# evfro/polara

Hardware: AMD Instinct MI355X
Metric: users scored/sec + SVD build time, ML-20M rank-50 PureSVD (higher is better)
Workload: dtype bf16x3; 1 GPU; ML-20M-shaped synthetic 138493 x 26744, ~2e7 nnz, 10 levels (BASELINE.json metric / configs[2]), PureSVD rank=50, top-10, all users scored; n_items=26744, nnz=19975287, rank=50, topk=10, prune=True, launch=python, passes on 2 streams

## Files before the change

include/polara_hip.h:

```cpp
#ifndef POLARA_HIP_H
#define POLARA_HIP_H

#include <stdint.h>

#ifdef __cplusplus
extern "C" {
#endif

#define PK_OK 0
#define PK_E_INVALID (-1)
#define PK_E_LAUNCH (-2)
#define PK_E_UNSUPPORTED (-3)
#define PK_E_NOCONV (-4)

#define PK_VAL_F32 0
#define PK_VAL_F64 1

const char *pk_last_error(void);
int pk_version(void);
int pk_set_option(const char *name, int32_t value, int32_t unset);
int pk_copy_to_host_async(void *stream, void *dst_host, const void *src_dev, int64_t bytes);
int pk_device_info(int device, char *name, int name_len, int *cu_count, int64_t *hbm_bytes);
int pk_warm_up(void);

// ... 171 lines not shown
                            const int64_t *task_end_dev, const int32_t *task_slot_dev, int64_t n_long,
                            const int32_t *long_row_dev, const int32_t *long_slot_begin_dev,
                            const int32_t *long_slot_end_dev, const int32_t *indices_dev, const void *vals_dev,
                            int val_kind, const double *X_dev, int64_t ldx, int32_t nc, double *out_dev, int64_t ldo,
                            double *partial_dev, int64_t x_rows, const int32_t *row_flags_dev, int32_t flag_mask);

int pk_spmm_csr_rows_list_f64(void *stream, int64_t cap, const int32_t *list_dev, const int32_t *count_dev, int64_t row_offset,
                              const int64_t *row_first_task_dev, const int32_t *task_row_dev, const int64_t *task_begin_dev,
                              const int64_t *task_end_dev, const int32_t *task_slot_dev, int64_t n_long,
                              const int32_t *long_row_dev, const int32_t *long_slot_begin_dev, const int32_t *long_slot_end_dev,
                              const int32_t *indices_dev, const void *vals_dev, int val_kind, const double *X_dev, int64_t ldx,
                              int32_t nc, double *out_dev, int64_t ldo, double *partial_dev, int64_t x_rows,
                              const int32_t *row_flags_dev, int32_t flag_mask);

int32_t pk_q20_lanes(int32_t K);
double pk_q20_kappa(int32_t K);
int64_t pk_q20_image_bytes(int64_t n, int32_t K);
int pk_q20_encode_f64(void *stream, int64_t n, int32_t K, const double *V_dev, int64_t ldv, void *img_dev,
                      double *tab_dev, void *work_dev, int32_t *info_dev);
int pk_q20_decode_f64(void *stream, int64_t n, int32_t K, const void *img_dev, const double *tab_dev, double *out_dev,
                      int64_t ldo);
int pk_fold_q20(void *stream, int64_t n_tasks, const int32_t *task_row_dev, const int64_t *task_begin_dev,
                const int64_t *task_end_dev, const int32_t *task_slot_dev, int64_t n_long,
                const int32_t *long_row_dev, const int32_t *long_slot_begin_dev, const int32_t *long_slot_end_dev,
                const int32_t *indices_dev, const void *vals_dev, int val_kind, const void *img_dev,
                const double *tab_dev, int64_t n_items, int32_t K, int32_t Kx, double *out_dev, int64_t ldo,
                double *partial_dev);
int pk_fold_q20_zero(void *stream, int64_t n_tasks, const int32_t *task_row_dev, const int64_t *task_begin_dev,
                     const int64_t *task_end_dev, const int32_t *task_slot_dev, int64_t n_long,
                     const int32_t *long_row_dev, const int32_t *long_slot_begin_dev, const int32_t *long_slot_end_dev,
                     const int32_t *indices_dev, const void *vals_dev, int val_kind, const void *img_dev,
                     const double *tab_dev, int64_t n_items, int32_t K, int32_t Kx, double *out_dev, int64_t ldo,
                     double *partial_dev, int32_t *zero_dev, int32_t zero_n);
int pk_scatter_rows_i64(void *stream, int64_t n_rows, int32_t width, const int64_t *src_dev, const int64_t *perm_dev,
                        int64_t *dst);
int pk_map_ids_i64(void *stream, int64_t n, const int64_t *src_dev, const int64_t *table_dev, int64_t n_table, int64_t *dst);
int64_t pk_exact_work_bytes(int32_t n_rows, int64_t n_items);
int pk_score_exact_rows_f64(void *stream, int32_t n_rows, const int32_t *rows_dev, int64_t n_items,
                            int32_t K, const double *V_dev, int64_t ldv, const double *E_dev, int64_t lde,
                            const int64_t *seen_ptr_dev, const int32_t *seen_idx_dev, int32_t topk,
                            int64_t *out_idx_dev, double *out_score_dev, void *work_dev);
int pk_exact_work_init(void *stream, void *work_dev, int32_t n_rows, int64_t n_items);
int pk_score_exact_list_f64(void *stream, int32_t n_wg, const int32_t *list_dev, const int32_t *count_dev, int64_t n_items,
                            int32_t K, const double *V_dev, int64_t ldv, const double *E_dev, int64_t lde,
                            const int64_t *seen_ptr_dev, const int32_t *seen_idx_dev, int32_t topk, int64_t *out_idx_dev,
                            double *out_score_dev, void *work_dev, const int64_t *out_perm_dev);
int pk_eval_ranks(void *stream, int64_t n_holdout, const int64_t *recs_dev, int32_t topk,
                  const int64_t *hold_row_dev, const int64_t *hold_item_dev, int32_t *rank_out_dev);
int32_t pk_eval_cols(void);
int pk_eval_user_metrics(void *stream, int64_t n_users, int32_t topk, const int64_t *recs_dev, int64_t ld,
                         const int64_t *hold_ptr_dev, const int64_t *hold_item_dev, const double *hold_rel_dev,
                         const unsigned char *hold_pos_dev, double not_rated_penalty, double switch_positive,
                         int32_t alternative, double *out_dev);
int64_t pk_eval_reduce_work_bytes(int64_t n_users);
int pk_eval_reduce(void *stream, int64_t n_users, const double *table_dev, double *sums_dev, void *work_dev);
int pk_unique_count_i64(void *stream, int64_t n, const int64_t *ids_dev, int64_t n_bins, int32_t *flags_dev,
                        int64_t *count_dev);
int pk_dense_scores_f64(void *stream, int32_t n_rows, int64_t n_items, int32_t K, const double *V_dev,
                        int64_t ldv, const double *E_dev, int64_t lde, double *out_dev, int64_t ldo);
int pk_topk_rows_f64(void *stream, int64_t n_rows, int64_t n_cols, const double *scores_dev, int64_t ld, int32_t topk,
                     int64_t *out_idx_dev);

int32_t pk_i2i_max_topk(void);
int32_t pk_i2i_window(void);
int32_t pk_i2i_build_window(void);
int64_t pk_i2i_ld(int64_t n_items);
// ... 302 lines not shown
```

polara_amd/_lib.py:

```python
import ctypes as C
import os

_HERE = os.path.dirname(os.path.abspath(__file__))
LIB_PATH = os.environ.get('POLARA_HIP_LIB') or os.path.join(_HERE, 'libpolarahip.so')

PK_VAL_F32, PK_VAL_F64 = 0, 1
PK_KNN_SCALE, PK_KNN_COSINE, PK_KNN_TANIMOTO = 0, 1, 2
PK_PMF_MAX_BLOCKS = 4096
PK_WARP_MAX_SAMPLED = 64
PK_SPLIT_ASCENDING, PK_SPLIT_RANDOM_LO, PK_SPLIT_NO_ORDER, PK_SPLIT_POS_ASCENDING = 1, 2, 4, 8

_vp, _i32, _i64, _f64 = C.c_void_p, C.c_int32, C.c_int64, C.c_double


class PkSweepSettle(C.Structure):
    _fields_ = [('topk', _i32), ('vmax', _f64), ('item_norm', _vp), ('out_idx', _vp), ('out_perm', _vp), ('flags', _vp),
                ('open_list', _vp), ('open_count', _vp)]


PROTOTYPES = {
    'pk_last_error': (C.c_char_p, []),
    'pk_version': (C.c_int, []),
    'pk_warm_up': (C.c_int, []),
    'pk_device_info': (C.c_int, [C.c_int, C.c_char_p, C.c_int, C.POINTER(C.c_int), C.POINTER(_i64)]),
# ... 43 lines not shown
    'pk_pack_frag_f32': (C.c_int, [_vp, _i64, _i32, _vp, _i64, _vp]),
    'pk_candidate_capacity': (_i32, [_i32]),
    'pk_score_state_bytes': (_i64, [_i64, _i32]),
    'pk_score_splits': (_i32, [_i64, _i32]),
    'pk_seen_tiles_build': (C.c_int, [_vp, _i64, _vp, _vp, _i32, _i64, _vp, _vp]),
    'pk_seen_tiles_max_unsorted_row': (_i32, []),
    'pk_score_candidates_f32': (C.c_int, [_vp, _i64, _i64, _i32, _vp, _vp, _vp, _vp, _i64, _vp, _i64, _f64, _vp, _vp, _vp, _vp,
                                          _i32, _i32, _vp, _vp, _vp, _i32, _vp, _vp, _vp, _i32, C.POINTER(PkSweepSettle)]),
    'pk_sweep_settles': (C.c_int, [_i32]),
    'pk_score_two_phase_plan': (C.c_int, [_i64, _i64, _i32, _vp, _vp]),
    'pk_score_two_phase_f32': (C.c_int, [_vp, _i64, _i64, _i32, _vp, _vp, _vp, _vp, _i64, _vp, _i64, _f64, _vp, _vp, _vp, _vp,
                                         _i32, _i32, _i32, _vp, _vp, _vp, _vp, _vp, _i32, _vp, _vp, _vp, _i32]),
    'pk_seen_dense_bytes': (_i64, [_i64, _i32]),
    'pk_seen_dense_build': (C.c_int, [_vp, _i64, _vp, _vp, _vp, _i32, _vp, _vp]),
    'pk_score_chunk_launches': (_i32, [_i64, _i32, _i32, _i32, _i32]),
    'pk_pack_frag_bound_f32': (C.c_int, [_vp, _i64, _i32, _vp, _i64, _vp, _vp, _vp, _i64, _f64]),
    'pk_row_norm_bound_f32': (C.c_int, [_vp, _i64, _i32, _vp, _i64, _vp]),
    'pk_tile_norm_bound_f32': (C.c_int, [_vp, _i64, _i32, _vp, _i64, _vp, _vp]),
    'pk_flag_compact': (C.c_int, [_vp, _i64, _vp, _i32, _vp, _vp]),
    'pk_fold_rows_f64': (C.c_int, [_vp, _i64, _vp, _vp, _i64, _vp, _vp, _vp, C.c_int, _vp, _i64, _i32, _vp, _i64]),
    'pk_spmm_csr_flagged_f64': (C.c_int, [_vp, _i64, _vp, _vp, _vp, _vp, _i64, _vp, _vp, _vp, _vp, _vp, C.c_int, _vp, _i64, _i32,
                                          _vp, _i64, _vp, _i64, _vp, _i32]),
    'pk_spmm_csr_rows_list_f64': (C.c_int, [_vp, _i64, _vp, _vp, _i64, _vp, _vp, _vp, _vp, _vp, _i64, _vp, _vp, _vp, _vp, _vp, C.c_int,
                                            _vp, _i64, _i32, _vp, _i64, _vp, _i64, _vp, _i32]),
    'pk_q20_lanes': (_i32, [_i32]),
    'pk_q20_kappa': (_f64, [_i32]),
    'pk_q20_image_bytes': (_i64, [_i64, _i32]),
    'pk_q20_encode_f64': (C.c_int, [_vp, _i64, _i32, _vp, _i64, _vp, _vp, _vp, _vp]),
    'pk_q20_decode_f64': (C.c_int, [_vp, _i64, _i32, _vp, _vp, _vp, _i64]),
    'pk_fold_q20': (C.c_int, [_vp, _i64, _vp, _vp, _vp, _vp, _i64, _vp, _vp, _vp, _vp, _vp, C.c_int, _vp, _vp, _i64, _i32, _i32,
                              _vp, _i64, _vp]),
    'pk_fold_q20_zero': (C.c_int, [_vp, _i64, _vp, _vp, _vp, _vp, _i64, _vp, _vp, _vp, _vp, _vp, C.c_int, _vp, _vp, _i64, _i32, _i32,
                                   _vp, _i64, _vp, _vp, _i32]),
    'pk_rescore_f64': (C.c_int, [_vp, _i64, _vp, _vp, _i64, _i64, _i32, _vp, _i64, _vp, _i64, _vp, _i64, _vp, _i64, _i32, _vp, _i32, _i32,
                                 _vp, _vp, _i32, _f64, _vp, _vp, _vp, _vp, _vp, _i32, _vp, _vp, _vp]),
    'pk_zero_i32': (C.c_int, [_vp, _vp, _i32]),
    'pk_scatter_rows_i64': (C.c_int, [_vp, _i64, _i32, _vp, _vp, _vp]),
    'pk_map_ids_i64': (C.c_int, [_vp, _i64, _vp, _vp, _i64, _vp]),
    'pk_exact_work_bytes': (_i64, [_i32, _i64]),
    'pk_score_exact_rows_f64': (C.c_int, [_vp, _i32, _vp, _i64, _i32, _vp, _i64, _vp, _i64, _vp, _vp, _i32,
                                          _vp, _vp, _vp]),
    'pk_score_exact_list_f64': (C.c_int, [_vp, _i32, _vp, _vp, _i64, _i32, _vp, _i64, _vp, _i64, _vp, _vp, _i32,
                                          _vp, _vp, _vp, _vp]),
    'pk_exact_work_init': (C.c_int, [_vp, _vp, _i32, _i64]),
    'pk_eval_ranks': (C.c_int, [_vp, _i64, _vp, _i32, _vp, _vp, _vp]),
    'pk_eval_cols': (_i32, []),
    'pk_eval_user_metrics': (C.c_int, [_vp, _i64, _i32, _vp, _i64, _vp, _vp, _vp, _vp, _f64, _f64, _i32, _vp]),
    'pk_eval_reduce_work_bytes': (_i64, [_i64]),
    'pk_eval_reduce': (C.c_int, [_vp, _i64, _vp, _vp, _vp]),
    'pk_unique_count_i64': (C.c_int, [_vp, _i64, _vp, _i64, _vp, _vp]),
    'pk_dense_scores_f64': (C.c_int, [_vp, _i32, _i64, _i32, _vp, _i64, _vp, _i64, _vp, _i64]),
    'pk_topk_rows_f64': (C.c_int, [_vp, _i64, _i64, _vp, _i64, _i32, _vp]),
    'pk_i2i_max_topk': (_i32, []),
    'pk_i2i_window': (_i32, []),
    'pk_i2i_build_window': (_i32, []),
    'pk_i2i_ld': (_i64, [_i64]),
    'pk_i2i_chunk_users': (_i64, [_i64, _i64, _i32]),
    'pk_i2i_topk_work_bytes': (_i64, [_i64, _i64, _i32]),
    'pk_i2i_build_f64': (C.c_int, [_vp, _i64, _i64, _vp, _vp, _vp, C.c_int, _vp, _vp, _vp, _vp, _i64]),
    'pk_i2i_image_f32': (C.c_int, [_vp, _i64, _vp, _vp, _vp]),
    'pk_i2i_topk': (C.c_int, [_vp, _i64, _i64, _vp, _vp, _vp, C.c_int, _vp, C.c_int, _i64, _i32, _i32, _i32, _vp, _vp, _vp]),
    'pk_spsp_topk_work_bytes': (_i64, [_i64, _i64, _i32]),
    'pk_spsp_topk': (C.c_int, [_vp, _i64, _i64, _i64, _vp, _vp, _vp, C.c_int, _vp, _vp, _vp, _i32, _i32, _i32, _vp, _vp, _vp]),
    'pk_spsp_topk_seen': (C.c_int, [_vp, _i64, _i64, _i64, _vp, _vp, _vp, C.c_int, _vp, _vp, _vp, _vp, _vp, _i32, _i32, _i32, _vp, _vp,
                                    _vp]),
    'pk_spsp_rows_f64': (C.c_int, [_vp, _i64, _i64, _i64, _i64, _vp, _vp, _vp, C.c_int, _vp, _vp, _vp, _vp, _i64]),
# ... 165 lines not shown
```

polara_amd/csrc/api.cpp:

```cpp
#include "pk_common.h"
#include <string.h>

static thread_local char g_err[512] = "";

void pk_set_error(const char *fmt, ...) {
    va_list ap;
    va_start(ap, fmt);
    vsnprintf(g_err, sizeof(g_err), fmt, ap);
    va_end(ap);
}

extern "C" const char *pk_last_error(void) { return g_err; }

#include <atomic>
namespace {
struct Option { const char *name; std::atomic<int> value; std::atomic<bool> set; };
Option g_options[] = {{"score_boot_tiles", {0}, {false}}, {"score_head_tiles", {0}, {false}}, {"score_phase2_splits", {0}, {false}},
                      {"rescore_settle", {0}, {false}}, {"sweep_settle", {0}, {false}}, {"slim_r_global", {0}, {false}}};
}
int pk_option(const char *name, int dflt) {
    for (auto &o : g_options)
        if (!strcmp(o.name, name)) return o.set.load() ? o.value.load() : dflt;
    return dflt;
}
extern "C" int pk_set_option(const char *name, int32_t value, int32_t unset) {
    if (name)
        for (auto &o : g_options)
            if (!strcmp(o.name, name)) {
                o.value.store(value);
                o.set.store(!unset);
                return PK_OK;
            }
    pk_set_error("pk_set_option: unknown option '%s'", name ? name : "(null)");
    return PK_E_INVALID;
}
extern "C" int pk_version(void) { return 104; }

extern "C" int pk_copy_to_host_async(void *stream, void *dst_host, const void *src_dev, int64_t bytes) {
    if (bytes < 0 || (bytes > 0 && (!dst_host || !src_dev))) {
        pk_set_error("pk_copy_to_host_async: bad arguments");
        return PK_E_INVALID;
    }
    if (bytes == 0) return PK_OK;
    const hipError_t e = hipMemcpyAsync(dst_host, src_dev, (size_t)bytes, hipMemcpyDeviceToHost, static_cast<hipStream_t>(stream));
    if (e != hipSuccess) {
        pk_set_error("pk_copy_to_host_async: %s", hipGetErrorString(e));
        return PK_E_LAUNCH;
    }
    return PK_OK;
}

extern "C" int pk_device_info(int device, char *name, int name_len, int *cu_count, int64_t *hbm_bytes) {
    int n = 0;
    hipError_t e = hipGetDeviceCount(&n);
    if (e != hipSuccess || n <= 0) {
        pk_set_error("pk_device_info: no HIP device visible (%s)", hipGetErrorString(e));
        return PK_E_LAUNCH;
    }
    if (device < 0 || device >= n) {
        pk_set_error("pk_device_info: device %d out of range [0,%d)", device, n);
        return PK_E_INVALID;
    }
    hipDeviceProp_t prop;
    e = hipGetDeviceProperties(&prop, device);
    if (e != hipSuccess) {
        pk_set_error("pk_device_info: %s", hipGetErrorString(e));
        return PK_E_LAUNCH;
    }
    if (name && name_len > 0) {
// ... 50 lines not shown
```

polara_amd/csrc/foldq.hip:

```cpp
#include "pk_common.h"
#include <math.h>
#include <stdlib.h>
#include <type_traits>

#define PK_Q20_TAB 96

__host__ __device__ __forceinline__ int pk_q20_bracket(unsigned j) {
    if (j < 4u) return (int)j;
#ifdef __HIP_DEVICE_COMPILE__
    const int e = 31 - __clz((int)j);
#else
    const int e = 31 - __builtin_clz(j);
#endif
    return 4 * (e - 1) + (int)((j >> (e - 2)) & 3u);
}

static inline int q20_lanes(int K) {
    if (K <= 12) return 2;
    if (K <= 25) return 4;
    if (K <= 50) return 8;
    if (K <= 101) return 16;
    if (K <= 202) return 32;
    return 0;
}
// ... 186 lines not shown

extern "C" int pk_q20_decode_f64(void *stream, int64_t n, int32_t K, const void *img_dev, const double *tab_dev, double *out_dev,
                                 int64_t ldo) {
    const int L = q20_lanes(K);
    PK_REQUIRE(L != 0 && n >= 1 && ldo >= K + 1, "pk_q20_decode_f64: bad sizes");
    hipStream_t st = pk_stream(stream);
    const dim3 grid((unsigned)pk_ceil_div(n * L, 256));
    const uint4 *img = static_cast<const uint4 *>(img_dev);
    const double kappa = q20_kappa(K);
    switch (L) {
        case 2: hipLaunchKernelGGL(q20_decode_kernel<2>, grid, dim3(256), 0, st, n, K, img, tab_dev, kappa, out_dev, ldo); break;
        case 4: hipLaunchKernelGGL(q20_decode_kernel<4>, grid, dim3(256), 0, st, n, K, img, tab_dev, kappa, out_dev, ldo); break;
        case 8: hipLaunchKernelGGL(q20_decode_kernel<8>, grid, dim3(256), 0, st, n, K, img, tab_dev, kappa, out_dev, ldo); break;
        case 16: hipLaunchKernelGGL(q20_decode_kernel<16>, grid, dim3(256), 0, st, n, K, img, tab_dev, kappa, out_dev, ldo); break;
        default: hipLaunchKernelGGL(q20_decode_kernel<32>, grid, dim3(256), 0, st, n, K, img, tab_dev, kappa, out_dev, ldo); break;
    }
    PK_CHECK_LAUNCH("q20_decode_kernel");
    return PK_OK;
}

__device__ __forceinline__ double q20_swap_add32(double x, double y) {
    const auto lo = __builtin_amdgcn_permlane32_swap((unsigned)__double2loint(x), (unsigned)__double2loint(y), false, false);
    const auto hi = __builtin_amdgcn_permlane32_swap((unsigned)__double2hiint(x), (unsigned)__double2hiint(y), false, false);
    return __hiloint2double((int)hi[0], (int)lo[0]) + __hiloint2double((int)hi[1], (int)lo[1]);
}
__device__ __forceinline__ double q20_swap_add16(double x, double y) {
    const auto lo = __builtin_amdgcn_permlane16_swap((unsigned)__double2loint(x), (unsigned)__double2loint(y), false, false);
    const auto hi = __builtin_amdgcn_permlane16_swap((unsigned)__double2hiint(x), (unsigned)__double2hiint(y), false, false);
    return __hiloint2double((int)hi[0], (int)lo[0]) + __hiloint2double((int)hi[1], (int)lo[1]);
}

typedef float pk_f2 __attribute__((ext_vector_type(2)));

template <typename VT, int L, int U>
__global__ __launch_bounds__(256) void fold_q20_kernel(
    int64_t n_tasks, const int32_t *__restrict__ task_row, const int64_t *__restrict__ task_begin,
    const int64_t *__restrict__ task_end, const int32_t *__restrict__ task_slot,
    const int32_t *__restrict__ indices, const VT *__restrict__ vals, const uint4 *__restrict__ img,
    const double *__restrict__ tab, double kappa, int K, int Kx, double *__restrict__ out, int64_t ldo,
    double *__restrict__ partial) {
    constexpr int GROUPS = 64 / L;
    constexpr int SPC = L;
    constexpr int SETS = SPC / U;
    static_assert(SETS >= 1 && SETS * U == SPC, "a chunk is a whole number of register sets");
    constexpr int LOG_RB = L == 2 ? 5 : (L == 4 ? 6 : (L == 8 ? 7 : (L == 16 ? 8 : 9)));
    const int lane = threadIdx.x & 63;
    const int wave = __builtin_amdgcn_readfirstlane((int)(threadIdx.x >> 6));
    const int64_t task = (int64_t)blockIdx.x * 4 + wave;
    if (task >= n_tasks) return;
    const int64_t p0 = task_begin[task];
    const int n = (int)(task_end[task] - p0);
    const int g = lane / L, l = lane % L;
    const int32_t *ip = indices + p0;
    const VT *vp = vals + p0;
    const char *Xb = reinterpret_cast<const char *>(img);
    const unsigned lo0 = (unsigned)l << 4;

    double acc[7];
#pragma unroll
    for (int t = 0; t < 7; ++t) acc[t] = 0.0;

    int jc = 0, jn = 0;
    VT araw = (VT)0, an = (VT)0;
    if (lane < n) {
        jc = ip[lane];
        araw = vp[lane];
    }
    if (64 + lane < n) {
        jn = ip[64 + lane];
        an = vp[64 + lane];
    }
    auto issue = [&](int jch, int st0, int cnt_ch, uint4(&x)[U]) {
#pragma unroll
        for (int u = 0; u < U; ++u) {
            if (u > 0 && (st0 + u) * GROUPS >= cnt_ch) break;
            const int jj = __shfl(jch, (st0 + u) * GROUPS + g, 64);
            unsigned off;
            asm("v_lshl_or_b32 %0, %1, %2, %3" : "=v"(off) : "v"(jj), "n"(LOG_RB), "v"(lo0));
            x[u] = *reinterpret_cast<const uint4 *>(Xb + off);
        }
    };
    auto consume = [&](float ach, int st0, int cnt_ch, const uint4(&x)[U]) {
        pk_f2 s01 = {0.0f, 0.0f}, s23 = {0.0f, 0.0f}, s45 = {0.0f, 0.0f};
        float s6 = 0.0f;
#pragma unroll
        for (int u = 0; u < U; ++u) {
            if (u > 0 && (st0 + u) * GROUPS >= cnt_ch) break;
            const float a = __shfl(ach, (st0 + u) * GROUPS + g, 64);
            const pk_f2 aa = {a, a};
            const uint4 d = x[u];
            const pk_f2 x01 = {(float)(int)__builtin_amdgcn_alignbit(d.x, d.y, 24), (float)(int)__builtin_amdgcn_alignbit(d.x, d.y, 4)};
            const pk_f2 x23 = {(float)(int)__builtin_amdgcn_alignbit(d.y, d.z, 16), (float)(int)__builtin_amdgcn_alignbit(d.z, d.w, 28)};
            const pk_f2 x45 = {(float)(int)__builtin_amdgcn_alignbit(d.z, d.w, 8), (float)(int)(d.w << 12)};
            s01 = __builtin_elementwise_fma(aa, x01, s01);
            s23 = __builtin_elementwise_fma(aa, x23, s23);
            s45 = __builtin_elementwise_fma(aa, x45, s45);
            s6 = fmaf(a, (float)(int)d.x, s6);
        }
        acc[0] += (double)s01.x;
        acc[1] += (double)s01.y;
        acc[2] += (double)s23.x;
        acc[3] += (double)s23.y;
        acc[4] += (double)s45.x;
        acc[5] += (double)s45.y;
        acc[6] += (double)s6;
    };
    uint4 x0[U], x1[U];
    issue(jc, 0, n < 64 ? n : 64, x0);
    float ac = (float)((double)araw * tab[pk_q20_bracket((unsigned)jc)]);
    auto chunk = [&](int p, auto P) {
        constexpr int P0 = decltype(P)::value;
        const int cnt = (n - p) < 64 ? (n - p) : 64;
        const bool more = p + 64 < n;
        const int cnt_next = (n - p - 64) < 64 ? (n - p - 64) : 64;
        int jf = 0;
        VT af = (VT)0;
        if (p + 128 + lane < n) {
            jf = ip[p + 128 + lane];
            af = vp[p + 128 + lane];
        }
        double sn = 0.0;
        if (more) sn = tab[pk_q20_bracket((unsigned)jn)];
#pragma unroll
        for (int k = 0; k < SETS; ++k) {
            const bool have = k * U * GROUPS < cnt;
            const bool have_next = (k + 1 < SETS) ? ((k + 1) * U * GROUPS < cnt) : more;
            if (((k + P0) & 1) == 0) {
                if (have_next) {
                    if (k + 1 < SETS) issue(jc, (k + 1) * U, cnt, x1);
                    else issue(jn, 0, cnt_next, x1);
                }
                if (have) consume(ac, k * U, cnt, x0);
            } else {
                if (have_next) {
                    if (k + 1 < SETS) issue(jc, (k + 1) * U, cnt, x0);
                    else issue(jn, 0, cnt_next, x0);
                }
                if (have) consume(ac, k * U, cnt, x1);
            }
        }
        jc = jn;
        ac = (float)((double)an * sn);
        jn = jf;
        an = af;
    };
    if constexpr ((SETS & 1) == 0) {
        for (int p = 0; p < n; p += 64) chunk(p, std::integral_constant<int, 0>());
    } else {
        for (int p = 0; p < n; p += 128) {
            chunk(p, std::integral_constant<int, 0>());
            if (p + 64 < n) chunk(p + 64, std::integral_constant<int, 1>());
        }
    }

    double w[4];
    w[0] = q20_swap_add32(acc[0], acc[4]);
    w[1] = q20_swap_add32(acc[1], acc[5]);
    w[2] = q20_swap_add32(acc[2], acc[6]);
    w[3] = q20_swap_add32(acc[3], 0.0);
    constexpr int NW = L <= 16 ? 2 : 4;
    if constexpr (L <= 16) {
        w[0] = q20_swap_add16(w[0], w[2]);
        w[1] = q20_swap_add16(w[1], w[3]);
    }
#pragma unroll
    for (int i = 0; i < NW; ++i) {
        if constexpr (L <= 8) w[i] += pk_lane_xor<8>(w[i]);
        if constexpr (L <= 4) w[i] += pk_lane_xor<4>(w[i]);
        if constexpr (L <= 2) w[i] += pk_lane_xor<2>(w[i]);
    }
    const int b5 = (lane >> 5) & 1, b4 = (lane >> 4) & 1;
    const int t0 = L <= 16 ? 4 * b5 + 2 * b4 : 4 * b5;
    const double dsum = L <= 16 ? w[0] : w[2];
    const double a1 = __shfl(dsum, lane + 1, 64), a2 = __shfl(dsum, lane + 2, 64);
    const int slot = task_slot[task];
    double *dst = slot < 0 ? out + (int64_t)task_row[task] * ldo : partial + (int64_t)slot * Kx;
    const bool owner = L <= 16 ? (((lane & 15) / L) == 0) : true;
    if (owner) {
#pragma unroll
        for (int i = 0; i < NW; ++i) {
            const int t = t0 + i;
            if (t < 6 && 6 * l + t < K) dst[6 * l + t] = w[i];
        }
        const bool digit_lane = L <= 16 ? (t0 == 6) : (b5 == 1);
        if (digit_lane) {
            const int e = l / 3;
            if (l % 3 == 0 && 3 * e + 2 <= L - 2 && 6 * L + e < K) dst[6 * L + e] = 2.0 * (dsum + a1 * 0.00390625 + a2 * 1.52587890625e-05);
            if (l == L - 1) {
                dst[K] = kappa * dsum;
                for (int c = K + 1; c < Kx; ++c) dst[c] = 0.0;
            }
        }
    }
}

__global__ __launch_bounds__(256) void fold_q20_fixup_kernel(int64_t n_long, const int32_t *__restrict__ long_row,
                                                             const int32_t *__restrict__ slot_begin, const int32_t *__restrict__ slot_end,
                                                             const double *__restrict__ partial, int nc, double *__restrict__ out, int64_t ldo,
                                                             int32_t *__restrict__ zero, int zero_n) {
    if (blockIdx.x == 0)
        for (int i = threadIdx.x; i < zero_n; i += blockDim.x) zero[i] = 0;
    const int64_t r = blockIdx.x;
    if (r >= n_long) return;
    const int s0 = slot_begin[r], s1 = slot_end[r];
    double *dst = out + (int64_t)long_row[r] * ldo;
    for (int c = threadIdx.x; c < nc; c += blockDim.x) {
        double a = 0.0;
        for (int s = s0; s < s1; ++s) a += partial[(int64_t)s * nc + c];
        dst[c] = a;
    }
}

template <typename VT>
static void launch_fold_q20(hipStream_t st, int L, int64_t n_tasks, const int32_t *task_row, const int64_t *task_begin,
                            const int64_t *task_end, const int32_t *task_slot, const int32_t *indices, const void *vals,
                            const uint4 *img, const double *tab, double kappa, int K, int Kx, double *out, int64_t ldo, double *partial) {
    const dim3 grid((unsigned)pk_ceil_div(n_tasks, 4)), block(256);
    const VT *v = static_cast<const VT *>(vals);
#define PK_FOLDQ(LL, UU)                                                                                                      \
    hipLaunchKernelGGL((fold_q20_kernel<VT, LL, UU>), grid, block, 0, st, n_tasks, task_row, task_begin, task_end, task_slot, \
                       indices, v, img, tab, kappa, K, Kx, out, ldo, partial)
    switch (L) {
        case 2: PK_FOLDQ(2, 1); break;
        case 4: PK_FOLDQ(4, 2); break;
        case 8:
            if (q20_steps(8) == 2) PK_FOLDQ(8, 2);
            else if (q20_steps(8) == 8) PK_FOLDQ(8, 8);
            else PK_FOLDQ(8, 4);
            break;
        case 16: PK_FOLDQ(16, 4); break;
        default: PK_FOLDQ(32, 4); break;
    }
#undef PK_FOLDQ
}

extern "C" int pk_fold_q20_zero(void *stream, int64_t n_tasks, const int32_t *task_row_dev, const int64_t *task_begin_dev,
                                const int64_t *task_end_dev, const int32_t *task_slot_dev, int64_t n_long,
                                const int32_t *long_row_dev, const int32_t *long_slot_begin_dev, const int32_t *long_slot_end_dev,
                                const int32_t *indices_dev, const void *vals_dev, int val_kind, const void *img_dev,
                                const double *tab_dev, int64_t n_items, int32_t K, int32_t Kx, double *out_dev, int64_t ldo,
                                double *partial_dev, int32_t *zero_dev, int32_t zero_n) {
    const int L = q20_lanes(K);
    PK_REQUIRE(L != 0 && n_tasks >= 0 && Kx >= K + 1 && ldo >= Kx, "pk_fold_q20: bad sizes (K=%d, Kx=%d)", K, Kx);
    PK_REQUIRE(n_items >= 1 && n_items < (1 << 24) && n_items * L * 16 < ((int64_t)1 << 32), "pk_fold_q20: image beyond 32-bit offsets");
    PK_REQUIRE(n_long == 0 || partial_dev != nullptr, "pk_fold_q20: partial buffer required");
    PK_REQUIRE(val_kind == PK_VAL_F32 || val_kind == PK_VAL_F64, "pk_fold_q20: bad val_kind %d", val_kind);
    PK_REQUIRE(zero_n >= 0 && zero_n <= (1 << 20) && (zero_n == 0 || zero_dev != nullptr), "pk_fold_q20: bad counter range");
    hipStream_t st = pk_stream(stream);
    if (n_tasks == 0) n_long = 0;
    if (n_tasks > 0) {
        const uint4 *img = static_cast<const uint4 *>(img_dev);
        const double kappa = q20_kappa(K);
        if (val_kind == PK_VAL_F32)
            launch_fold_q20<float>(st, L, n_tasks, task_row_dev, task_begin_dev, task_end_dev, task_slot_dev, indices_dev, vals_dev, img,
                                   tab_dev, kappa, K, Kx, out_dev, ldo, partial_dev);
        else
            launch_fold_q20<double>(st, L, n_tasks, task_row_dev, task_begin_dev, task_end_dev, task_slot_dev, indices_dev, vals_dev, img,
                                    tab_dev, kappa, K, Kx, out_dev, ldo, partial_dev);
        PK_CHECK_LAUNCH("fold_q20_kernel");
    }
    if (n_long > 0 || zero_n > 0) {
        hipLaunchKernelGGL(fold_q20_fixup_kernel, dim3((unsigned)(n_long > 0 ? n_long : 1)), dim3(256), 0, st, n_long, long_row_dev,
                           long_slot_begin_dev, long_slot_end_dev, partial_dev, Kx, out_dev, ldo, zero_dev, (int)zero_n);
        PK_CHECK_LAUNCH("fold_q20_fixup_kernel");
    }
    return PK_OK;
}

extern "C" int pk_fold_q20(void *stream, int64_t n_tasks, const int32_t *task_row_dev, const int64_t *task_begin_dev,
                           const int64_t *task_end_dev, const int32_t *task_slot_dev, int64_t n_long,
                           const int32_t *long_row_dev, const int32_t *long_slot_begin_dev, const int32_t *long_slot_end_dev,
                           const int32_t *indices_dev, const void *vals_dev, int val_kind, const void *img_dev,
                           const double *tab_dev, int64_t n_items, int32_t K, int32_t Kx, double *out_dev, int64_t ldo,
                           double *partial_dev) {
    return pk_fold_q20_zero(stream, n_tasks, task_row_dev, task_begin_dev, task_end_dev, task_slot_dev, n_long, long_row_dev,
                            long_slot_begin_dev, long_slot_end_dev, indices_dev, vals_dev, val_kind, img_dev, tab_dev, n_items, K, Kx,
                            out_dev, ldo, partial_dev, nullptr, 0);
}

hipError_t pk_tu_load_foldq() {
    hipFuncAttributes a;
    return hipFuncGetAttributes(&a, reinterpret_cast<const void *>(&q20_scale_kernel));
}
```

polara_amd/ops.py:

```python
import ctypes as C

import numpy as np
import torch

from . import _lib
from .csr import SPLIT_NNZ


_PTR_KEEP = None


def _ptr(t, offset=0):
    if t is None:
        return None
    if _PTR_KEEP is not None:
        _PTR_KEEP.append(t)
    return C.c_void_p(t.data_ptr() + offset * t.element_size())


def _raw_stream(index):
    return torch._C._cuda_getCurrentRawStream(index)


class _KernelTimer:
    __slots__ = ('ops', 'name', 'meta', 'e0', 'e1')

    def __init__(self, ops, name, meta):
        self.ops, self.name, self.meta = ops, name, meta

    def __enter__(self):
        if self.ops.timers is not None:
            self.e0 = torch.cuda.Event(enable_timing=True)
            self.e1 = torch.cuda.Event(enable_timing=True)
            self.e0.record(torch.cuda.current_stream(self.ops.device))

    def __exit__(self, *exc):
        if self.ops.timers is not None:
            self.e1.record(torch.cuda.current_stream(self.ops.device))
            self.ops.timers.setdefault(self.name, []).append((self.e0, self.e1, self.meta))
        return False

# ... 564 lines not shown
        return flags

    def csr_transpose(self, A, rows_per_block=0):
        n_rows, n_cols = A.shape
        nnz = int(A.indices.numel())
        n_blocks = -(-n_rows // rows_per_block) if rows_per_block else 1
        t_indptr = torch.empty(n_blocks * n_cols + 1, dtype=torch.int64, device=self.device)
        t_indices = torch.empty(max(nnz, 1), dtype=torch.int32, device=self.device)[:nnz]
        t_values = torch.empty(max(nnz, 1), dtype=A.values.dtype, device=self.device)[:nnz]
        work = self._work(self.lib.pk_csr_transpose_work_bytes(nnz))
        with self._timed('transpose', (n_rows, n_cols, nnz)):
            _lib.check(self.lib.pk_csr_transpose(self.stream(), n_rows, n_cols, nnz, _ptr(A.indptr), _ptr(A.indices),
                                                 _ptr(A.values), A.val_kind, int(rows_per_block), _ptr(t_indptr),
                                                 _ptr(t_indices), _ptr(t_values), _ptr(work)), 'pk_csr_transpose')
        T = DeviceCSR.from_device(self, t_indptr, t_indices, t_values, (n_blocks * n_cols, n_rows), A.split)
        T._nnz = nnz
        return T

    def csr_rows_by_length(self, A):
        n_rows = A.shape[0]
        nnz = int(A.indices.numel())
        perm = torch.empty(n_rows, dtype=torch.int32, device=self.device)
        indptr = torch.empty(n_rows + 1, dtype=torch.int64, device=self.device)
        idx = torch.empty_like(A.indices)
        val = torch.empty_like(A.values)
        work = self._work(self.lib.pk_csr_rows_by_length_work_bytes(n_rows))
        _lib.check(self.lib.pk_csr_rows_by_length(self.stream(), n_rows, nnz, _ptr(A.indptr), _ptr(A.indices), _ptr(A.values),
                                                  A.val_kind, _ptr(perm), _ptr(indptr), _ptr(idx), _ptr(val), _ptr(work)),
                   'pk_csr_rows_by_length')
        P = DeviceCSR.from_device(self, indptr, idx, val, A.shape, A.split)
        P._nnz = nnz
        P.sorted_cols = A.sorted_cols
        P._nonneg = getattr(A, '_nonneg', None)
        return P, perm.long()

    def csr_relabel_cols(self, A, col_map, sort=True):
        dev = self.device
        if torch.is_tensor(col_map):
            cm = col_map.to(device=dev, dtype=torch.int32)
        else:
            cm = torch.as_tensor(np.ascontiguousarray(col_map, dtype=np.int32)).to(dev)
        if not sort:
            new = A.with_columns(cm[A.indices.long()], A.values)
            new.sorted_cols = False
            return new
        nnz = int(A.indices.numel())
        idx = torch.empty_like(A.indices)
        val = torch.empty_like(A.values)
        work = self._work(self.lib.pk_csr_relabel_work_bytes(nnz))
        _lib.check(self.lib.pk_csr_relabel_sorted(self.stream(), A.shape[0], A.shape[1], nnz, _ptr(A.indptr), _ptr(A.indices),
                                                  _ptr(A.values), A.val_kind, _ptr(cm.contiguous()), _ptr(idx), _ptr(val),
                                                  _ptr(work)), 'pk_csr_relabel_sorted')
        new = A.with_columns(idx, val)
        new.sorted_cols = True
        return new

    def csr_scale(self, A, row_scale, col_scale):
        rs = torch.as_tensor(np.ascontiguousarray(row_scale, dtype=np.float64)).to(self.device) if not torch.is_tensor(row_scale) else row_scale
        cs = torch.as_tensor(np.ascontiguousarray(col_scale, dtype=np.float64)).to(self.device) if not torch.is_tensor(col_scale) else col_scale
        assert rs.numel() == A.shape[0] and cs.numel() == A.shape[1]
        out = torch.empty(max(int(A.indices.numel()), 1), dtype=torch.float64, device=self.device)[:A.indices.numel()]
        _lib.check(self.lib.pk_csr_scale_f64(self.stream(), A.shape[0], _ptr(A.indptr), _ptr(A.indices), _ptr(A.values), A.val_kind,
                                             _ptr(rs), _ptr(cs), _ptr(out)), 'pk_csr_scale_f64')
        new = A.with_columns(A.indices, out)
        new.val_kind = _lib.PK_VAL_F64
        return new
# ... 148 lines not shown
    def spmm_flagged_ok(self, X):
        return X.dtype == torch.float64 and X.shape[1] % 2 == 0 and X.stride(0) % 2 == 0 and X.data_ptr() % 16 == 0 and 2 <= X.shape[1] <= 256

    def q20_supported(self, n_items, K):
        L = self.lib.pk_q20_lanes(int(K))
        return L != 0 and n_items < (1 << 24) and n_items * L * 16 < (1 << 32)

    def q20_encode(self, V):
        assert V.stride(1) == 1 and V.dtype == torch.float64
        n, K = V.shape
        if not self.q20_supported(n, K):
            return None
        nbytes = self.lib.pk_q20_image_bytes(n, K)
        raw = torch.empty(nbytes + 128, dtype=torch.uint8, device=self.device)
        off = (-raw.data_ptr()) % 128
        img = raw[off:off + nbytes].view(n, nbytes // n)
        tab = torch.empty(96, dtype=torch.float64, device=self.device)
        work = torch.empty(768, dtype=torch.uint8, device=self.device)
        info = torch.empty(1, dtype=torch.int32, device=self.device)
        _lib.check(self.lib.pk_q20_encode_f64(self.stream(), n, K, _ptr(V), V.stride(0), _ptr(img), _ptr(tab), _ptr(work),
                                              _ptr(info)), 'pk_q20_encode_f64')
        if int(info.item()) != 0:
            return None
        return img, tab

    def q20_decode(self, image, K):
        img, tab = image
        n = img.shape[0]
        out = self.empty(n, K + 1)
        _lib.check(self.lib.pk_q20_decode_f64(self.stream(), n, K, _ptr(img), _ptr(tab), _ptr(out), out.stride(0)),
                   'pk_q20_decode_f64')
        return out

    def fold_q20(self, A, image, K, out, rows=None, counters=None):
        img, tab = image
        Kx = out.shape[1]
        assert out.dtype == torch.float64 and out.stride(1) == 1 and Kx >= K + 1 and img.shape[0] == A.shape[1]
        t0, n_tasks, l0, n_long = (0, A.n_tasks, 0, A.n_long) if rows is None else A.task_range(int(rows[0]), int(rows[1]))
        p = A.plan
        meta = None
        if self.timers is not None:
            meta = (A.shape[0], A.shape[1], A.nnz, Kx, A.values.element_size(), img.shape[1])
        args = (self.stream(), n_tasks, _ptr(p['task_row'], t0), _ptr(p['task_begin'], t0), _ptr(p['task_end'], t0),
                _ptr(p['task_slot'], t0), n_long, _ptr(p['long_row'], l0), _ptr(p['long_slot_begin'], l0),
                _ptr(p['long_slot_end'], l0), _ptr(A.indices), _ptr(A.values), A.val_kind, _ptr(img), _ptr(tab),
                int(A.shape[1]), int(K), int(Kx), _ptr(out), out.stride(0), _ptr(A.partial(Kx)))
        with self._timed('fold_q20', meta):
            if counters is None:
                _lib.check(self.lib.pk_fold_q20(*args), 'pk_fold_q20')
            else:
                assert counters.dtype == torch.int32 and counters.is_contiguous() and counters.numel() >= 1
                _lib.check(self.lib.pk_fold_q20_zero(*args, _ptr(counters), int(counters.numel())), 'pk_fold_q20_zero')
        return out

    def fold_q20_zero(self, A, image, K, out, n_counters, rows=None):
        c = torch.empty(int(n_counters), dtype=torch.int32, device=self.device)
        self.fold_q20(A, image, K, out, rows=rows, counters=c)
        return c

    def gram(self, A, B=None):
        B = A if B is None else B
        assert A.stride(1) == 1 and B.stride(1) == 1 and A.shape[0] == B.shape[0]
        n, la = A.shape
        lb = B.shape[1]
        need = self.lib.pk_gram_work_bytes(n, la, lb)
        key = self.stream_key()
        if self._gram_work is None:
            self._gram_work = {}
        work = self._gram_work.get(key)
        if work is None or work.numel() * 8 < need:
            work = self._gram_work[key] = self.empty((need + 7) // 8)
        G = self.empty(la, lb)
        _lib.check(self.lib.pk_gram_f64(self.stream(), n, la, lb, _ptr(A), A.stride(0), _ptr(B), B.stride(0),
                                        _ptr(G), G.stride(0), _ptr(work)), 'pk_gram_f64')
        return G

    def tsmm(self, X, Cm, out=None):
        assert X.stride(1) == 1 and Cm.stride(1) == 1 and Cm.shape[0] == X.shape[1]
        n, lin = X.shape
        lout = Cm.shape[1]
        if out is None:
            out = self.empty(n, lout)
        _lib.check(self.lib.pk_tsmm_f64(self.stream(), n, lin, lout, _ptr(X), X.stride(0), _ptr(Cm), Cm.stride(0),
                                        _ptr(out), out.stride(0)), 'pk_tsmm_f64')
        return out

# ... 1728 lines not shown
```

Baseline: 203.5 million users/s.

## Pack multiple short fold tasks per wavefront in q20 fold kernel

Adds a tasks-per-wave template parameter so one 64-lane wave can process 2 or 4 adjacent CSR row tasks, each in a lane slice, instead of one task per wave. For short rows, a single task left most lanes and shuffle slots idle. Slices run to the longest row among the packed tasks. The Python side enables this only for row-permuted matrices marked as having similar adjacent lengths, and only when there are enough tasks to fill the device. The cost is wasted work when packed rows differ in length, plus a different reduction path.

Measured after the change: 207.8 million users/s, median of 6. 2.1% higher.

```diff
diff --git a/include/polara_hip.h b/include/polara_hip.h
--- a/include/polara_hip.h
+++ b/include/polara_hip.h
@@ -227,6 +227,12 @@
                      const int32_t *indices_dev, const void *vals_dev, int val_kind, const void *img_dev,
                      const double *tab_dev, int64_t n_items, int32_t K, int32_t Kx, double *out_dev, int64_t ldo,
                      double *partial_dev, int32_t *zero_dev, int32_t zero_n);
+int pk_fold_q20_sliced(void *stream, int64_t n_tasks, const int32_t *task_row_dev, const int64_t *task_begin_dev,
+                       const int64_t *task_end_dev, const int32_t *task_slot_dev, int64_t n_long,
+                       const int32_t *long_row_dev, const int32_t *long_slot_begin_dev, const int32_t *long_slot_end_dev,
+                       const int32_t *indices_dev, const void *vals_dev, int val_kind, const void *img_dev,
+                       const double *tab_dev, int64_t n_items, int32_t K, int32_t Kx, double *out_dev, int64_t ldo,
+                       double *partial_dev, int32_t *zero_dev, int32_t zero_n, int32_t tasks_per_wave);
 int pk_scatter_rows_i64(void *stream, int64_t n_rows, int32_t width, const int64_t *src_dev, const int64_t *perm_dev,
                         int64_t *dst);
 int pk_map_ids_i64(void *stream, int64_t n, const int64_t *src_dev, const int64_t *table_dev, int64_t n_table, int64_t *dst);
diff --git a/polara_amd/_lib.py b/polara_amd/_lib.py
--- a/polara_amd/_lib.py
+++ b/polara_amd/_lib.py
@@ -99,6 +99,8 @@
                               _vp, _i64, _vp]),
     'pk_fold_q20_zero': (C.c_int, [_vp, _i64, _vp, _vp, _vp, _vp, _i64, _vp, _vp, _vp, _vp, _vp, C.c_int, _vp, _vp, _i64, _i32, _i32,
                                    _vp, _i64, _vp, _vp, _i32]),
+    'pk_fold_q20_sliced': (C.c_int, [_vp, _i64, _vp, _vp, _vp, _vp, _i64, _vp, _vp, _vp, _vp, _vp, C.c_int, _vp, _vp, _i64, _i32, _i32,
+                                     _vp, _i64, _vp, _vp, _i32, _i32]),
     'pk_rescore_f64': (C.c_int, [_vp, _i64, _vp, _vp, _i64, _i64, _i32, _vp, _i64, _vp, _i64, _vp, _i64, _vp, _i64, _i32, _vp, _i32, _i32,
                                  _vp, _vp, _i32, _f64, _vp, _vp, _vp, _vp, _vp, _i32, _vp, _vp, _vp]),
     'pk_zero_i32': (C.c_int, [_vp, _vp, _i32]),
diff --git a/polara_amd/csrc/api.cpp b/polara_amd/csrc/api.cpp
--- a/polara_amd/csrc/api.cpp
+++ b/polara_amd/csrc/api.cpp
@@ -34,7 +34,7 @@
     pk_set_error("pk_set_option: unknown option '%s'", name ? name : "(null)");
     return PK_E_INVALID;
 }
-extern "C" int pk_version(void) { return 104; }
+extern "C" int pk_version(void) { return 105; }
 
 extern "C" int pk_copy_to_host_async(void *stream, void *dst_host, const void *src_dev, int64_t bytes) {
     if (bytes < 0 || (bytes > 0 && (!dst_host || !src_dev))) {
diff --git a/polara_amd/csrc/foldq.hip b/polara_amd/csrc/foldq.hip
--- a/polara_amd/csrc/foldq.hip
+++ b/polara_amd/csrc/foldq.hip
@@ -242,7 +242,7 @@
 
 typedef float pk_f2 __attribute__((ext_vector_type(2)));
 
-template <typename VT, int L, int U>
+template <typename VT, int L, int U, int T>
 __global__ __launch_bounds__(256) void fold_q20_kernel(
     int64_t n_tasks, const int32_t *__restrict__ task_row, const int64_t *__restrict__ task_begin,
     const int64_t *__restrict__ task_end, const int32_t *__restrict__ task_slot,
@@ -250,17 +250,38 @@
     const double *__restrict__ tab, double kappa, int K, int Kx, double *__restrict__ out, int64_t ldo,
     double *__restrict__ partial) {
     constexpr int GROUPS = 64 / L;
+    constexpr int GS = GROUPS / T;
+    constexpr int CH = 64 / T;
     constexpr int SPC = L;
     constexpr int SETS = SPC / U;
+    static_assert(T == 1 || T == 2 || T == 4, "1, 2 or 4 tasks per wave");
+    static_assert(GS >= 2 && GS * T == GROUPS, "a slice holds at least two lane groups");
     static_assert(SETS >= 1 && SETS * U == SPC, "a chunk is a whole number of register sets");
     constexpr int LOG_RB = L == 2 ? 5 : (L == 4 ? 6 : (L == 8 ? 7 : (L == 16 ? 8 : 9)));
     const int lane = threadIdx.x & 63;
     const int wave = __builtin_amdgcn_readfirstlane((int)(threadIdx.x >> 6));
-    const int64_t task = (int64_t)blockIdx.x * 4 + wave;
-    if (task >= n_tasks) return;
-    const int64_t p0 = task_begin[task];
-    const int n = (int)(task_end[task] - p0);
+    const int64_t wtask = ((int64_t)blockIdx.x * 4 + wave) * T;
+    if (wtask >= n_tasks) return;
+    const int sl = T == 1 ? 0 : lane / CH, ls = lane % CH;
+    const int64_t task = wtask + sl;
+    const bool real = T == 1 || task < n_tasks;
+    int64_t p0 = 0;
+    int n = 0;
+    if (real) {
+        p0 = task_begin[task];
+        n = (int)(task_end[task] - p0);
+    }
+    int nmax = n;
+    if constexpr (T > 1) {
+        nmax = __builtin_amdgcn_readlane(n, 0);
+#pragma unroll
+        for (int s = 1; s < T; ++s) {
+            const int ns = __builtin_amdgcn_readlane(n, s * CH);
+            nmax = ns > nmax ? ns : nmax;
+        }
+    }
     const int g = lane / L, l = lane % L;
+    const int src0 = T == 1 ? g : (lane & ~(CH - 1)) | (g % GS);
     const int32_t *ip = indices + p0;
     const VT *vp = vals + p0;
     const char *Xb = reinterpret_cast<const char *>(img);
@@ -272,19 +293,19 @@
 
     int jc = 0, jn = 0;
     VT araw = (VT)0, an = (VT)0;
-    if (lane < n) {
-        jc = ip[lane];
-        araw = vp[lane];
-    }
-    if (64 + lane < n) {
-        jn = ip[64 + lane];
-        an = vp[64 + lane];
+    if (ls < n) {
+        jc = ip[ls];
+        araw = vp[ls];
+    }
+    if (CH + ls < n) {
+        jn = ip[CH + ls];
+        an = vp[CH + ls];
     }
     auto issue = [&](int jch, int st0, int cnt_ch, uint4(&x)[U]) {
 #pragma unroll
         for (int u = 0; u < U; ++u) {
-            if (u > 0 && (st0 + u) * GROUPS >= cnt_ch) break;
-            const int jj = __shfl(jch, (st0 + u) * GROUPS + g, 64);
+            if (u > 0 && (st0 + u) * GS >= cnt_ch) break;
+            const int jj = __shfl(jch, (st0 + u) * GS + src0, 64);
             unsigned off;
             asm("v_lshl_or_b32 %0, %1, %2, %3" : "=v"(off) : "v"(jj), "n"(LOG_RB), "v"(lo0));
             x[u] = *reinterpret_cast<const uint4 *>(Xb + off);
@@ -295,8 +316,8 @@
         float s6 = 0.0f;
 #pragma unroll
         for (int u = 0; u < U; ++u) {
-            if (u > 0 && (st0 + u) * GROUPS >= cnt_ch) break;
-            const float a = __shfl(ach, (st0 + u) * GROUPS + g, 64);
+            if (u > 0 && (st0 + u) * GS >= cnt_ch) break;
+            const float a = __shfl(ach, (st0 + u) * GS + src0, 64);
             const pk_f2 aa = {a, a};
             const uint4 d = x[u];
             const pk_f2 x01 = {(float)(int)__builtin_amdgcn_alignbit(d.x, d.y, 24), (float)(int)__builtin_amdgcn_alignbit(d.x, d.y, 4)};
@@ -316,25 +337,25 @@
         acc[6] += (double)s6;
     };
     uint4 x0[U], x1[U];
-    issue(jc, 0, n < 64 ? n : 64, x0);
+    issue(jc, 0, nmax < CH ? nmax : CH, x0);
     float ac = (float)((double)araw * tab[pk_q20_bracket((unsigned)jc)]);
     auto chunk = [&](int p, auto P) {
         constexpr int P0 = decltype(P)::value;
-        const int cnt = (n - p) < 64 ? (n - p) : 64;
-        const bool more = p + 64 < n;
-        const int cnt_next = (n - p - 64) < 64 ? (n - p - 64) : 64;
+        const int cnt = (nmax - p) < CH ? (nmax - p) : CH;
+        const bool more = p + CH < nmax;
+        const int cnt_next = (nmax - p - CH) < CH ? (nmax - p - CH) : CH;
         int jf = 0;
         VT af = (VT)0;
-        if (p + 128 + lane < n) {
-            jf = ip[p + 128 + lane];
-            af = vp[p + 128 + lane];
+        if (p + 2 * CH + ls < n) {
+            jf = ip[p + 2 * CH + ls];
+            af = vp[p + 2 * CH + ls];
         }
         double sn = 0.0;
         if (more) sn = tab[pk_q20_bracket((unsigned)jn)];
 #pragma unroll
         for (int k = 0; k < SETS; ++k) {
-            const bool have = k * U * GROUPS < cnt;
-            const bool have_next = (k + 1 < SETS) ? ((k + 1) * U * GROUPS < cnt) : more;
+            const bool have = k * U * GS < cnt;
+            const bool have_next = (k + 1 < SETS) ? ((k + 1) * U * GS < cnt) : more;
             if (((k + P0) & 1) == 0) {
                 if (have_next) {
                     if (k + 1 < SETS) issue(jc, (k + 1) * U, cnt, x1);
@@ -355,23 +376,33 @@
         an = af;
     };
     if constexpr ((SETS & 1) == 0) {
-        for (int p = 0; p < n; p += 64) chunk(p, std::integral_constant<int, 0>());
+        for (int p = 0; p < nmax; p += CH) chunk(p, std::integral_constant<int, 0>());
     } else {
-        for (int p = 0; p < n; p += 128) {
+        for (int p = 0; p < nmax; p += 2 * CH) {
             chunk(p, std::integral_constant<int, 0>());
-            if (p + 64 < n) chunk(p + 64, std::integral_constant<int, 1>());
-        }
-    }
-
-    double w[4];
-    w[0] = q20_swap_add32(acc[0], acc[4]);
-    w[1] = q20_swap_add32(acc[1], acc[5]);
-    w[2] = q20_swap_add32(acc[2], acc[6]);
-    w[3] = q20_swap_add32(acc[3], 0.0);
-    constexpr int NW = L <= 16 ? 2 : 4;
-    if constexpr (L <= 16) {
-        w[0] = q20_swap_add16(w[0], w[2]);
-        w[1] = q20_swap_add16(w[1], w[3]);
+            if (p + CH < nmax) chunk(p + CH, std::integral_constant<int, 1>());
+        }
+    }
+
+    constexpr int NW = T == 4 ? 7 : ((T == 2 || L == 32) ? 4 : 2);
+    double w[NW];
+    if constexpr (T == 1) {
+        const double h0 = q20_swap_add32(acc[0], acc[4]), h1 = q20_swap_add32(acc[1], acc[5]);
+        const double h2 = q20_swap_add32(acc[2], acc[6]), h3 = q20_swap_add32(acc[3], 0.0);
+        if constexpr (L <= 16) {
+            w[0] = q20_swap_add16(h0, h2);
+            w[1] = q20_swap_add16(h1, h3);
+        } else {
+            w[0] = h0, w[1] = h1, w[2] = h2, w[3] = h3;
+        }
+    } else if constexpr (T == 2) {
+        w[0] = q20_swap_add16(acc[0], acc[4]);
+        w[1] = q20_swap_add16(acc[1], acc[5]);
+        w[2] = q20_swap_add16(acc[2], acc[6]);
+        w[3] = q20_swap_add16(acc[3], 0.0);
+    } else {
+#pragma unroll
+        for (int i = 0; i < 7; ++i) w[i] = acc[i];
     }
 #pragma unroll
     for (int i = 0; i < NW; ++i) {
@@ -380,19 +411,25 @@
         if constexpr (L <= 2) w[i] += pk_lane_xor<2>(w[i]);
     }
     const int b5 = (lane >> 5) & 1, b4 = (lane >> 4) & 1;
-    const int t0 = L <= 16 ? 4 * b5 + 2 * b4 : 4 * b5;
-    const double dsum = L <= 16 ? w[0] : w[2];
+    const int t0 = T == 4 ? 0 : (T == 2 ? 4 * b4 : (L <= 16 ? 4 * b5 + 2 * b4 : 4 * b5));
+    constexpr int DW = T == 4 ? 6 : ((T == 2 || L == 32) ? 2 : 0);
+    const double dsum = w[DW];
     const double a1 = __shfl(dsum, lane + 1, 64), a2 = __shfl(dsum, lane + 2, 64);
-    const int slot = task_slot[task];
-    double *dst = slot < 0 ? out + (int64_t)task_row[task] * ldo : partial + (int64_t)slot * Kx;
-    const bool owner = L <= 16 ? (((lane & 15) / L) == 0) : true;
+    int slot = -1;
+    int64_t row = 0;
+    if (real) {
+        slot = task_slot[task];
+        row = task_row[task];
+    }
+    double *dst = slot < 0 ? out + row * ldo : partial + (int64_t)slot * Kx;
+    const bool owner = real && (L <= 16 ? (((lane & 15) / L) == 0) : true);
     if (owner) {
 #pragma unroll
         for (int i = 0; i < NW; ++i) {
             const int t = t0 + i;
             if (t < 6 && 6 * l + t < K) dst[6 * l + t] = w[i];
         }
-        const bool digit_lane = L <= 16 ? (t0 == 6) : (b5 == 1);
+        const bool digit_lane = T == 4 ? true : (T == 2 ? (b4 == 1) : (L <= 16 ? (t0 == 6) : (b5 == 1)));
         if (digit_lane) {
             const int e = l / 3;
             if (l % 3 == 0 && 3 * e + 2 <= L - 2 && 6 * L + e < K) dst[6 * L + e] = 2.0 * (dsum + a1 * 0.00390625 + a2 * 1.52587890625e-05);
@@ -422,26 +459,72 @@
 }
 
 template <typename VT>
-static void launch_fold_q20(hipStream_t st, int L, int64_t n_tasks, const int32_t *task_row, const int64_t *task_begin,
+static void launch_fold_q20(hipStream_t st, int L, int T, int64_t n_tasks, const int32_t *task_row, const int64_t *task_begin,
                             const int64_t *task_end, const int32_t *task_slot, const int32_t *indices, const void *vals,
                             const uint4 *img, const double *tab, double kappa, int K, int Kx, double *out, int64_t ldo, double *partial) {
-    const dim3 grid((unsigned)pk_ceil_div(n_tasks, 4)), block(256);
+    const dim3 grid((unsigned)pk_ceil_div(n_tasks, (int64_t)4 * T)), block(256);
     const VT *v = static_cast<const VT *>(vals);
-#define PK_FOLDQ(LL, UU)                                                                                                      \
-    hipLaunchKernelGGL((fold_q20_kernel<VT, LL, UU>), grid, block, 0, st, n_tasks, task_row, task_begin, task_end, task_slot, \
+#define PK_FOLDQ(LL, UU, TT)                                                                                                      \
+    hipLaunchKernelGGL((fold_q20_kernel<VT, LL, UU, TT>), grid, block, 0, st, n_tasks, task_row, task_begin, task_end, task_slot, \
                        indices, v, img, tab, kappa, K, Kx, out, ldo, partial)
+#define PK_FOLDQ_T4(LL, UU)                      \
+    do {                                         \
+        if (T == 4) PK_FOLDQ(LL, UU, 4);         \
+        else if (T == 2) PK_FOLDQ(LL, UU, 2);    \
+        else PK_FOLDQ(LL, UU, 1);                \
+    } while (0)
     switch (L) {
-        case 2: PK_FOLDQ(2, 1); break;
-        case 4: PK_FOLDQ(4, 2); break;
+        case 2: PK_FOLDQ_T4(2, 1); break;
+        case 4: PK_FOLDQ_T4(4, 2); break;
         case 8:
-            if (q20_steps(8) == 2) PK_FOLDQ(8, 2);
-            else if (q20_steps(8) == 8) PK_FOLDQ(8, 8);
-            else PK_FOLDQ(8, 4);
+            if (q20_steps(8) == 2) PK_FOLDQ_T4(8, 2);
+            else if (q20_steps(8) == 8) PK_FOLDQ_T4(8, 8);
+            else PK_FOLDQ_T4(8, 4);
             break;
-        case 16: PK_FOLDQ(16, 4); break;
-        default: PK_FOLDQ(32, 4); break;
-    }
+        case 16:
+            if (T == 2) PK_FOLDQ(16, 4, 2);
+            else PK_FOLDQ(16, 4, 1);
+            break;
+        default: PK_FOLDQ(32, 4, 1); break;
+    }
+#undef PK_FOLDQ_T4
 #undef PK_FOLDQ
+}
+
+extern "C" int pk_fold_q20_sliced(void *stream, int64_t n_tasks, const int32_t *task_row_dev, const int64_t *task_begin_dev,
+                                  const int64_t *task_end_dev, const int32_t *task_slot_dev, int64_t n_long,
+                                  const int32_t *long_row_dev, const int32_t *long_slot_begin_dev, const int32_t *long_slot_end_dev,
+                                  const int32_t *indices_dev, const void *vals_dev, int val_kind, const void *img_dev,
+                                  const double *tab_dev, int64_t n_items, int32_t K, int32_t Kx, double *out_dev, int64_t ldo,
+                                  double *partial_dev, int32_t *zero_dev, int32_t zero_n, int32_t tasks_per_wave) {
+    const int L = q20_lanes(K);
+    PK_REQUIRE(L != 0 && n_tasks >= 0 && Kx >= K + 1 && ldo >= Kx, "pk_fold_q20: bad sizes (K=%d, Kx=%d)", K, Kx);
+    PK_REQUIRE(n_items >= 1 && n_items < (1 << 24) && n_items * L * 16 < ((int64_t)1 << 32), "pk_fold_q20: image beyond 32-bit offsets");
+    PK_REQUIRE(n_long == 0 || partial_dev != nullptr, "pk_fold_q20: partial buffer required");
+    PK_REQUIRE(val_kind == PK_VAL_F32 || val_kind == PK_VAL_F64, "pk_fold_q20: bad val_kind %d", val_kind);
+    PK_REQUIRE(zero_n >= 0 && zero_n <= (1 << 20) && (zero_n == 0 || zero_dev != nullptr), "pk_fold_q20: bad counter range");
+    PK_REQUIRE(tasks_per_wave == 1 || tasks_per_wave == 2 || tasks_per_wave == 4, "pk_fold_q20_sliced: tasks_per_wave %d (1, 2 or 4)",
+               tasks_per_wave);
+    const int T = L == 32 ? 1 : (L == 16 && tasks_per_wave > 2 ? 2 : tasks_per_wave);
+    hipStream_t st = pk_stream(stream);
+    if (n_tasks == 0) n_long = 0;
+    if (n_tasks > 0) {
+        const uint4 *img = static_cast<const uint4 *>(img_dev);
+        const double kappa = q20_kappa(K);
+        if (val_kind == PK_VAL_F32)
+            launch_fold_q20<float>(st, L, T, n_tasks, task_row_dev, task_begin_dev, task_end_dev, task_slot_dev, indices_dev, vals_dev,
+                                   img, tab_dev, kappa, K, Kx, out_dev, ldo, partial_dev);
+        else
+            launch_fold_q20<double>(st, L, T, n_tasks, task_row_dev, task_begin_dev, task_end_dev, task_slot_dev, indices_dev, vals_dev,
+                                    img, tab_dev, kappa, K, Kx, out_dev, ldo, partial_dev);
+        PK_CHECK_LAUNCH("fold_q20_kernel");
+    }
+    if (n_long > 0 || zero_n > 0) {
+        hipLaunchKernelGGL(fold_q20_fixup_kernel, dim3((unsigned)(n_long > 0 ? n_long : 1)), dim3(256), 0, st, n_long, long_row_dev,
+                           long_slot_begin_dev, long_slot_end_dev, partial_dev, Kx, out_dev, ldo, zero_dev, (int)zero_n);
+        PK_CHECK_LAUNCH("fold_q20_fixup_kernel");
+    }
+    return PK_OK;
 }
 
 extern "C" int pk_fold_q20_zero(void *stream, int64_t n_tasks, const int32_t *task_row_dev, const int64_t *task_begin_dev,
@@ -450,31 +533,9 @@
                                 const int32_t *indices_dev, const void *vals_dev, int val_kind, const void *img_dev,
                                 const double *tab_dev, int64_t n_items, int32_t K, int32_t Kx, double *out_dev, int64_t ldo,
                                 double *partial_dev, int32_t *zero_dev, int32_t zero_n) {
-    const int L = q20_lanes(K);
-    PK_REQUIRE(L != 0 && n_tasks >= 0 && Kx >= K + 1 && ldo >= Kx, "pk_fold_q20: bad sizes (K=%d, Kx=%d)", K, Kx);
-    PK_REQUIRE(n_items >= 1 && n_items < (1 << 24) && n_items * L * 16 < ((int64_t)1 << 32), "pk_fold_q20: image beyond 32-bit offsets");
-    PK_REQUIRE(n_long == 0 || partial_dev != nullptr, "pk_fold_q20: partial buffer required");
-    PK_REQUIRE(val_kind == PK_VAL_F32 || val_kind == PK_VAL_F64, "pk_fold_q20: bad val_kind %d", val_kind);
-    PK_REQUIRE(zero_n >= 0 && zero_n <= (1 << 20) && (zero_n == 0 || zero_dev != nullptr), "pk_fold_q20: bad counter range");
-    hipStream_t st = pk_stream(stream);
-    if (n_tasks == 0) n_long = 0;
-    if (n_tasks > 0) {
-        const uint4 *img = static_cast<const uint4 *>(img_dev);
-        const double kappa = q20_kappa(K);
-        if (val_kind == PK_VAL_F32)
-            launch_fold_q20<float>(st, L, n_tasks, task_row_dev, task_begin_dev, task_end_dev, task_slot_dev, indices_dev, vals_dev, img,
-                                   tab_dev, kappa, K, Kx, out_dev, ldo, partial_dev);
-        else
-            launch_fold_q20<double>(st, L, n_tasks, task_row_dev, task_begin_dev, task_end_dev, task_slot_dev, indices_dev, vals_dev, img,
-                                    tab_dev, kappa, K, Kx, out_dev, ldo, partial_dev);
-        PK_CHECK_LAUNCH("fold_q20_kernel");
-    }
-    if (n_long > 0 || zero_n > 0) {
-        hipLaunchKernelGGL(fold_q20_fixup_kernel, dim3((unsigned)(n_long > 0 ? n_long : 1)), dim3(256), 0, st, n_long, long_row_dev,
-                           long_slot_begin_dev, long_slot_end_dev, partial_dev, Kx, out_dev, ldo, zero_dev, (int)zero_n);
-        PK_CHECK_LAUNCH("fold_q20_fixup_kernel");
-    }
-    return PK_OK;
+    return pk_fold_q20_sliced(stream, n_tasks, task_row_dev, task_begin_dev, task_end_dev, task_slot_dev, n_long, long_row_dev,
+                              long_slot_begin_dev, long_slot_end_dev, indices_dev, vals_dev, val_kind, img_dev, tab_dev, n_items, K, Kx,
+                              out_dev, ldo, partial_dev, zero_dev, zero_n, 1);
 }
 
 extern "C" int pk_fold_q20(void *stream, int64_t n_tasks, const int32_t *task_row_dev, const int64_t *task_begin_dev,
@@ -483,9 +544,9 @@
                            const int32_t *indices_dev, const void *vals_dev, int val_kind, const void *img_dev,
                            const double *tab_dev, int64_t n_items, int32_t K, int32_t Kx, double *out_dev, int64_t ldo,
                            double *partial_dev) {
-    return pk_fold_q20_zero(stream, n_tasks, task_row_dev, task_begin_dev, task_end_dev, task_slot_dev, n_long, long_row_dev,
-                            long_slot_begin_dev, long_slot_end_dev, indices_dev, vals_dev, val_kind, img_dev, tab_dev, n_items, K, Kx,
-                            out_dev, ldo, partial_dev, nullptr, 0);
+    return pk_fold_q20_sliced(stream, n_tasks, task_row_dev, task_begin_dev, task_end_dev, task_slot_dev, n_long, long_row_dev,
+                              long_slot_begin_dev, long_slot_end_dev, indices_dev, vals_dev, val_kind, img_dev, tab_dev, n_items, K, Kx,
+                              out_dev, ldo, partial_dev, nullptr, 0, 1);
 }
 
 hipError_t pk_tu_load_foldq() {
diff --git a/polara_amd/ops.py b/polara_amd/ops.py
--- a/polara_amd/ops.py
+++ b/polara_amd/ops.py
@@ -7,6 +7,8 @@
 from .csr import SPLIT_NNZ
 
 
+FOLD_TASKS_PER_WAVE = 4
+FOLD_SLICED_MIN_WAVES = 25
 _PTR_KEEP = None
 
 
@@ -637,6 +639,7 @@
         P._nnz = nnz
         P.sorted_cols = A.sorted_cols
         P._nonneg = getattr(A, '_nonneg', None)
+        P.adjacent_alike = True
         return P, perm.long()
 
     def csr_relabel_cols(self, A, col_map, sort=True):
@@ -851,11 +854,13 @@
                    'pk_q20_decode_f64')
         return out
 
-    def fold_q20(self, A, image, K, out, rows=None, counters=None):
+    def fold_q20(self, A, image, K, out, rows=None, counters=None, tasks_per_wave=None):
         img, tab = image
         Kx = out.shape[1]
         assert out.dtype == torch.float64 and out.stride(1) == 1 and Kx >= K + 1 and img.shape[0] == A.shape[1]
         t0, n_tasks, l0, n_long = (0, A.n_tasks, 0, A.n_long) if rows is None else A.task_range(int(rows[0]), int(rows[1]))
+        if tasks_per_wave is None:
+            tasks_per_wave = self.fold_tasks_per_wave(A, n_tasks)
         p = A.plan
         meta = None
         if self.timers is not None:
@@ -864,13 +869,27 @@
                 _ptr(p['task_slot'], t0), n_long, _ptr(p['long_row'], l0), _ptr(p['long_slot_begin'], l0),
                 _ptr(p['long_slot_end'], l0), _ptr(A.indices), _ptr(A.values), A.val_kind, _ptr(img), _ptr(tab),
                 int(A.shape[1]), int(K), int(Kx), _ptr(out), out.stride(0), _ptr(A.partial(Kx)))
+        if counters is not None:
+            assert counters.dtype == torch.int32 and counters.is_contiguous() and counters.numel() >= 1
         with self._timed('fold_q20', meta):
-            if counters is None:
+            if tasks_per_wave != 1:
+                zero = (None, 0) if counters is None else (_ptr(counters), int(counters.numel()))
+                _lib.check(self.lib.pk_fold_q20_sliced(*args, *zero, int(tasks_per_wave)), 'pk_fold_q20_sliced')
+            elif counters is None:
                 _lib.check(self.lib.pk_fold_q20(*args), 'pk_fold_q20')
             else:
-                assert counters.dtype == torch.int32 and counters.is_contiguous() and counters.numel() >= 1
                 _lib.check(self.lib.pk_fold_q20_zero(*args, _ptr(counters), int(counters.numel())), 'pk_fold_q20_zero')
         return out
+
+    def fold_tasks_per_wave(self, A, n_tasks):
+        if not getattr(A, 'adjacent_alike', False):
+            return 1
+        if getattr(self, '_simds', None) is None:
+            self._simds = 4 * torch.cuda.get_device_properties(self.device).multi_processor_count
+        T = FOLD_TASKS_PER_WAVE
+        while T > 1 and n_tasks < T * FOLD_SLICED_MIN_WAVES * self._simds:
+            T //= 2
+        return T
 
     def fold_q20_zero(self, A, image, K, out, n_counters, rows=None):
         c = torch.empty(int(n_counters), dtype=torch.int32, device=self.device)
```
